# LukasHedegaard/continual-skeletons

Hardware: AMD Instinct MI355X
Metric: clips/sec (ST-GCN clip forward, NTU-60 shape; CoST-GCN online step reported under costgcn_online) (higher is better)
Workload: dtype f32

## Files before the change

### continual-skeletons_amd/csrc/tcn_wino.hip

```cpp
#include <type_traits>

#include "mfma_core.h"
#include "tcn_params.h"

namespace {

constexpr int WMT = 64;
constexpr int WNT = 128;
constexpr int WTAPS = 12;

template <int VT, int MW = 1>
constexpr int wino_ldb() { return ((2 * ((WNT / MW + VT - 2) / VT) + 10) * VT + 3) / 4 * 4; }

struct WStage12x64 {
    unsigned goff0, loff0, gstride;
    f32x4 v[6];
    __device__ __forceinline__ void setup(int Cpad, int Mpad, int tid) {
        goff0 = (unsigned)(((tid >> 7) * Cpad + ((tid >> 4) & 7)) * Mpad + (tid & 15) * 4);
        loff0 = (unsigned)(tid * 4);
        gstride = (unsigned)(2 * Cpad * Mpad);
    }
    __device__ __forceinline__ void issue_slot(int u, const float *__restrict__ chunk_base) {
        v[u] = *reinterpret_cast<const f32x4 *>(chunk_base + (size_t)u * gstride + goff0);
    }
    __device__ __forceinline__ void issue(const float *__restrict__ chunk_base) {
#pragma unroll
        for (int u = 0; u < 6; ++u) issue_slot(u, chunk_base);
    }
    template <int G>
    __device__ __forceinline__ void issue_part(const float *__restrict__ chunk_base) {
        issue_slot(2 * G, chunk_base);
        issue_slot(2 * G + 1, chunk_base);
    }
    __device__ __forceinline__ void commit(float *__restrict__ Wl) const {
#pragma unroll
        for (int u = 0; u < 6; ++u) *reinterpret_cast<f32x4 *>(Wl + u * (NTHREADS * 4) + loff0) = v[u];
    }
};

template <int NT>
struct WStageNx128 {
    unsigned goff0, loff0, gstride;
    f32x4 v[NT];
    __device__ __forceinline__ void setup(int Cpad, int Mpad, int tid) {
        goff0 = 4u * (unsigned)((tid >> 5) * Mpad + (tid & 31) * 4);
        loff0 = (unsigned)(tid * 4);
        gstride = (unsigned)(Cpad * Mpad);
    }
    __device__ __forceinline__ void issue_slot(int u, const float *__restrict__ chunk_base) {
        v[u] = *reinterpret_cast<const f32x4 *>(reinterpret_cast<const char *>(chunk_base + (size_t)u * gstride) + goff0);
    }
    __device__ __forceinline__ void issue(const float *__restrict__ chunk_base) {
#pragma unroll
        for (int u = 0; u < NT; ++u) issue_slot(u, chunk_base);
    }
    template <int G>
    __device__ __forceinline__ void issue_part(const float *__restrict__ chunk_base) {
        constexpr int lo = NT == 13 ? (G == 0 ? 0 : 3 * G + 1) : 4 * G, hi = NT == 13 ? 3 * G + 4 : 4 * G + 4;
#pragma unroll
        for (int u = lo; u < hi; ++u) issue_slot(u, chunk_base);
    }
    __device__ __forceinline__ void commit(float *__restrict__ Wl) const {
#pragma unroll
        for (int u = 0; u < NT; ++u) *reinterpret_cast<f32x4 *>(Wl + u * (KC * 128) + loff0) = v[u];
    }
};

struct WStageRes64 {
    unsigned goff0, loff0;
    f32x4 v;
    __device__ __forceinline__ void setup(int Mpad, int tid) {
        goff0 = (unsigned)(((tid >> 4) & 7) * Mpad + (tid & 15) * 4);
        loff0 = (unsigned)((tid & 127) * 4);
    }
    __device__ __forceinline__ void issue(const float *__restrict__ chunk_base) {
        v = *reinterpret_cast<const f32x4 *>(chunk_base + goff0);
    }
    __device__ __forceinline__ void commit(float *__restrict__ Wl) const { *reinterpret_cast<f32x4 *>(Wl + loff0) = v; }
};

struct WStageRes128 {
    unsigned goff0, loff0;
    f32x4 v;
    __device__ __forceinline__ void setup(int Mpad, int tid) {
        goff0 = (unsigned)((tid >> 5) * Mpad + (tid & 31) * 4);
        loff0 = (unsigned)(tid * 4);
    }
    __device__ __forceinline__ void issue(const float *__restrict__ chunk_base) {
        v = *reinterpret_cast<const f32x4 *>(chunk_base + goff0);
    }
    __device__ __forceinline__ void commit(float *__restrict__ Wl) const { *reinterpret_cast<f32x4 *>(Wl + loff0) = v; }
};

template <int VT, int G, int MW>
__device__ __forceinline__ void wino_group(const float *__restrict__ Wl, const float *__restrict__ Bl, int off, int l31, int kh,
                                           f32x16 (&acc)[4][2]) {
    constexpr int LDB = wino_ldb<VT, MW>(), MT = WMT * MW;
    const float *br = Bl + kh * LDB + off + 3 * G * VT;
    const float *wr = Wl + 4 * G * (KC * MT) + kh * MT + l31;
#pragma unroll
    for (int s = 0; s < KC / 2; ++s) {
        const float d0 = br[2 * s * LDB], d1 = br[2 * s * LDB + VT], d2 = br[2 * s * LDB + 2 * VT], d3 = br[2 * s * LDB + 3 * VT];
        const float b[4] = {d0 - d2, d1 + d2, d2 - d1, d1 - d3};
#pragma unroll
        for (int i = 0; i < 4; ++i) {
            const float a0 = wr[i * (KC * MT) + 2 * s * MT], a1 = wr[i * (KC * MT) + 2 * s * MT + 32];
            acc[i][0] = __builtin_amdgcn_mfma_f32_32x32x2f32(a0, b[i], acc[i][0], 0, 0, 0);
            acc[i][1] = __builtin_amdgcn_mfma_f32_32x32x2f32(a1, b[i], acc[i][1], 0, 0, 0);
        }
    }
}

template <int VT, int MW>
__device__ __forceinline__ void wino_valid_res_chunk(const float *__restrict__ Wl, const float *__restrict__ Bl, int off, int l31,
                                                     int kh, f32x16 (&acc)[4][2]) {
    constexpr int LDB = wino_ldb<VT, MW>(), MT = WMT * MW;
    const float *br = Bl + kh * LDB + off;
    const float *wr = Wl + kh * MT + l31;
#pragma unroll
    for (int s = 0; s < KC / 2; ++s) {
        const float d0 = br[2 * s * LDB], nd1 = -br[2 * s * LDB + VT];
        const float a0 = wr[2 * s * MT], a1 = wr[2 * s * MT + 32];
        acc[0][0] = __builtin_amdgcn_mfma_f32_32x32x2f32(a0, d0, acc[0][0], 0, 0, 0);
        acc[0][1] = __builtin_amdgcn_mfma_f32_32x32x2f32(a1, d0, acc[0][1], 0, 0, 0);
        acc[3][0] = __builtin_amdgcn_mfma_f32_32x32x2f32(a0, nd1, acc[3][0], 0, 0, 0);
        acc[3][1] = __builtin_amdgcn_mfma_f32_32x32x2f32(a1, nd1, acc[3][1], 0, 0, 0);
    }
}

template <int VT, bool RES, bool VALID = false>
__device__ __forceinline__ void wino_epilogue(const TcnParams &p, const f32x16 (&acc)[4][2], int m0, int q0, int qend, int seg,
                                              int wn, int l31, int kh, int jc, int vc) {
    const int T = p.Tout, TV = T * VT;
    const int TVR = VALID ? p.Tin * VT : TV;
    const bool qv = q0 + wn * 32 + l31 < qend;
    const bool odd_ok = 2 * jc + 1 < T;
    const unsigned p0 = (unsigned)(2 * jc * VT + vc);
    const unsigned b0 = 4u * (4u * (unsigned)kh * (unsigned)TV + p0);
    const unsigned b1 = odd_ok ? b0 + 4u * VT : b0;
    const unsigned kh16 = 16u * (unsigned)kh;
    const unsigned r0 = VALID ? 4u * (4u * (unsigned)kh * (unsigned)TVR + p0 + 4u * VT) : b0;
    const unsigned r1 = VALID ? (odd_ok ? r0 + 4u * VT : r0) : b1;
    const float *rseg = RES ? p.xres + (int64_t)seg * p.Cout * TVR : nullptr;
    float *oseg = p.out + (int64_t)seg * p.Cout * TV;
#pragma unroll
    for (int mi = 0; mi < 2; ++mi) {
        const int rb = m0 + mi * 32;
        float o0[16], o1[16];
#pragma unroll
        for (int g = 0; g < 16; ++g) {
            const int row = rb + (g & 3) + 8 * (g >> 2);
            const float bias = ld_lane(p.bias + row, kh16);
            const float m1 = acc[1][mi][g], m2 = acc[2][mi][g];
            float v0 = acc[0][mi][g] + m1 + m2 + bias;
            float v1 = m1 - m2 - acc[3][mi][g] + bias;
            if (RES) {
                const float *rrow = rseg + (int64_t)row * TVR;
                v0 += ld_lane(rrow, r0);
                v1 += ld_lane(rrow, r1);
            }
            if (p.relu) { v0 = relu_nan(v0); v1 = relu_nan(v1); }
            o0[g] = v0;
            o1[g] = v1;
        }
        if (qv) {
#pragma unroll
            for (int g = 0; g < 16; ++g) {
                float *orow = oseg + (int64_t)(rb + (g & 3) + 8 * (g >> 2)) * TV;
                st_lane(orow, b0, o0[g]);
                if (odd_ok) st_lane(orow, b1, o1[g]);
            }
        }
    }
}

}

template <int VT, bool RES = true, int MW = 1, bool VALID = false, bool RESCONV = false>
__global__ __launch_bounds__(NTHREADS, 2) void tcn_stage_wino_kernel(const TcnParams p) {
    static_assert(!RESCONV || (VALID && !RES), "the conv-residual phase is built for the valid form");
    constexpr int LDB = wino_ldb<VT, MW>(), MT = WMT * MW, NT = WNT / MW;
    constexpr int NJ = (LDB + 63) / 64;
    extern __shared__ __attribute__((aligned(16))) float smem[];
    float *Wl = smem;
    float *Bl = smem + WTAPS * KC * MT;

    const int tid = threadIdx.x, lane = tid & 63, wave = __builtin_amdgcn_readfirstlane(tid >> 6);
    const int l31 = lane & 31, kh = lane >> 5;
    const int wm = MW == 2 ? wave >> 1 : 0, wn = MW == 2 ? wave & 1 : wave;
    const unsigned wid = xcd_contiguous_id(blockIdx.x, gridDim.x);
    const int m0 = (int)(wid % p.mtiles) * MT, q0 = (int)((wid / p.mtiles) % p.qtiles) * NT;
    const int seg = (int)(wid / (p.mtiles * p.qtiles));
    const int T = VALID ? p.Tin : p.Tout, TV = T * VT, QP = p.nt;
    const int qend = min(q0 + NT, QP);
    const int ja = div_magic(q0, p.vmagic), jb = div_magic(qend - 1, p.vmagic);

    const int qc = min(q0 + wn * 32 + l31, qend - 1);
    const int jc = div_magic(qc, p.vmagic), vc = qc - jc * VT;
    const int off = 2 * (jc - ja) * VT + vc;

    f32x16 acc[4][2];
#pragma unroll
    for (int i = 0; i < 4; ++i)
#pragma unroll
        for (int mi = 0; mi < 2; ++mi)
#pragma unroll
            for (int g = 0; g < 16; ++g) acc[i][mi][g] = 0.f;

    {
        const int fa = VALID ? 2 * ja : 2 * ja - 4;
        const int span = (2 * (jb - ja) + 10) * VT;
        const int64_t cs = (int64_t)TV;
        const float *seg_base = p.y + (int64_t)seg * p.C * cs;
        const float *wbase = p.w + m0;
        const float *Ww = Wl + wm * WMT;
        std::conditional_t<MW == 2, WStageNx128<WTAPS>, WStage12x64> ws;
        ws.setup(p.Cpad, p.Mpad, tid);
        auto kloop = [&](auto &bx) {
            ws.issue(wbase);
            bx.issue(seg_base, p.C, cs, 0, wave);
            for (int c0 = 0; c0 + KC < p.Cpad; c0 += KC) {
                __syncthreads();
                ws.commit(Wl);
                bx.commit(Bl, LDB, wave);
                __syncthreads();
                const float *wnext = wbase + (size_t)(c0 + KC) * p.Mpad;
                const int cn = c0 + KC;
                ws.template issue_part<0>(wnext);
                bx.template issue_third<0>(seg_base, p.C, cs, cn, wave);
                __builtin_amdgcn_s_setprio(1);
                wino_group<VT, 0, MW>(Ww, Bl, off, l31, kh, acc);
                __builtin_amdgcn_s_setprio(0);
                ws.template issue_part<1>(wnext);
                bx.template issue_third<1>(seg_base, p.C, cs, cn, wave);
                __builtin_amdgcn_s_setprio(1);
                wino_group<VT, 1, MW>(Ww, Bl, off, l31, kh, acc);
                __builtin_amdgcn_s_setprio(0);
                ws.template issue_part<2>(wnext);
                bx.template issue_third<2>(seg_base, p.C, cs, cn, wave);
                __builtin_amdgcn_s_setprio(1);
                wino_group<VT, 2, MW>(Ww, Bl, off, l31, kh, acc);
                __builtin_amdgcn_s_setprio(0);
            }
            __syncthreads();
            ws.commit(Wl);
            bx.commit(Bl, LDB, wave);
            __syncthreads();
            wino_group<VT, 0, MW>(Ww, Bl, off, l31, kh, acc);
            wino_group<VT, 1, MW>(Ww, Bl, off, l31, kh, acc);
            wino_group<VT, 2, MW>(Ww, Bl, off, l31, kh, acc);
        };
        const bool interior = fa >= 0 && fa * VT + 4 * ((span + 3) / 4) <= TV;
        if (interior) {
            BStage4<(NJ + 3) / 4> b4;
            b4.setup(fa * VT, span, lane);
            kloop(b4);
        } else {
            BStage<NJ> bs;
            bs.setup(fa * VT, span, TV, lane);
            kloop(bs);
        }
    }

    if (RESCONV) {
        constexpr int NJ4R = (((2 * ((NT + VT - 2) / VT) + 2) * VT + 3) / 4 + 63) / 64;
        const int span = (2 * (jb - ja) + 2) * VT;
        const int64_t cs = (int64_t)p.Tres * VT;
        const float *seg_base = p.xres + (int64_t)seg * p.Cres * cs;
        const float *wbase = p.wres + m0;
        const float *Ww = Wl + wm * WMT;
        std::conditional_t<MW == 2, WStageRes128, WStageRes64> wr;
        wr.setup(p.Mpad, tid);
        BStage4<NJ4R> b4;
        b4.setup((2 * ja + 4) * VT, span, lane);
        wr.issue(wbase);
        b4.issue(seg_base, p.Cres, cs, 0, wave);
        for (int c0 = 0; c0 + KC < p.Cres; c0 += KC) {
            __syncthreads();
            wr.commit(Wl);
            b4.commit(Bl, LDB, wave);
            __syncthreads();
            wr.issue(wbase + (size_t)(c0 + KC) * p.Mpad);
            b4.issue(seg_base, p.Cres, cs, c0 + KC, wave);
            wino_valid_res_chunk<VT, MW>(Ww, Bl, off, l31, kh, acc);
        }
        __syncthreads();
        wr.commit(Wl);
        b4.commit(Bl, LDB, wave);
        __syncthreads();
        wino_valid_res_chunk<VT, MW>(Ww, Bl, off, l31, kh, acc);
    }

    wino_epilogue<VT, RES, VALID>(p, acc, m0 + wm * WMT, q0, qend, seg, wn, l31, kh, jc, vc);
}

namespace {

constexpr int W2TAPS = 13;

template <int VT, int MW = 1>
constexpr int wino2_ldb() { return ((4 * ((WNT / MW + VT - 2) / VT) + 11) * VT + 3) / 4 * 4; }

struct WStage13x64 {
    unsigned goff0, loff0, gstride, u6;
    f32x4 v[7];
    __device__ __forceinline__ void setup(int Cpad, int Mpad, int tid) {
        goff0 = (unsigned)(((tid >> 7) * Cpad + ((tid >> 4) & 7)) * Mpad + (tid & 15) * 4);
        loff0 = (unsigned)(tid * 4);
        gstride = (unsigned)(2 * Cpad * Mpad);
        u6 = tid >= 128 ? 5u : 6u;
    }
    __device__ __forceinline__ void issue_slot(int u, const float *__restrict__ chunk_base) {
        if (u < 6) v[u] = *reinterpret_cast<const f32x4 *>(chunk_base + (size_t)u * gstride + goff0);
        else v[6] = *reinterpret_cast<const f32x4 *>(chunk_base + (size_t)u6 * gstride + goff0);
    }
    __device__ __forceinline__ void issue(const float *__restrict__ chunk_base) {
#pragma unroll
        for (int u = 0; u < 7; ++u) issue_slot(u, chunk_base);
    }
    template <int G>
    __device__ __forceinline__ void issue_part(const float *__restrict__ chunk_base) {
        if (G < 3) {
            issue_slot(2 * G, chunk_base);
            issue_slot(2 * G + 1, chunk_base);
        } else {
            issue_slot(6, chunk_base);
        }
    }
    __device__ __forceinline__ void commit(float *__restrict__ Wl) const {
#pragma unroll
        for (int u = 0; u < 6; ++u) *reinterpret_cast<f32x4 *>(Wl + u * (NTHREADS * 4) + loff0) = v[u];
        *reinterpret_cast<f32x4 *>(Wl + u6 * (NTHREADS * 4) + loff0) = v[6];
    }
};

template <int LDB>
struct BStage4Tail {
    static constexpr int RPW = KC / (NTHREADS / 64);
    static constexpr int REST = LDB % 256;
    static constexpr int NV = LDB / 256 + (REST > 128 ? 1 : 0), NS = REST > 128 ? 0 : (REST + 63) / 64;
    static_assert(NV >= 1 && NV <= 2 && NS <= 2, "issue_third: 16-byte sweeps with thirds 0 and 1, 4-byte sweeps with third 2");
    unsigned off4[NV], off1[NS > 0 ? NS : 1];
    int pbase_;
    f32x4 v[RPW][NV];
    float t[RPW][NS > 0 ? NS : 1];
    __device__ __forceinline__ void setup(int pbase, int span, int lane) {
        const int nvec = (span + 3) / 4;
        pbase_ = pbase;
#pragma unroll
        for (int u = 0; u < NV; ++u) off4[u] = (unsigned)(4 * min(u * 64 + lane, nvec - 1));
#pragma unroll
        for (int u = 0; u < NS; ++u) off1[u] = (unsigned)min(NV * 256 + u * 64 + lane, span - 1);
    }
    __device__ __forceinline__ const float *row(const float *__restrict__ seg_base, int C, int64_t chan_stride, int c0, int wave,
                                                int rr) const {
        const int c = min(c0 + wave + rr * (NTHREADS / 64), C - 1);
        return seg_base + (int64_t)c * chan_stride + pbase_;
    }
    template <int G>
    __device__ __forceinline__ void issue_third(const float *__restrict__ seg_base, int C, int64_t chan_stride, int c0, int wave) {
#pragma unroll
        for (int rr = 0; rr < RPW; ++rr) {
            const float *src = row(seg_base, C, chan_stride, c0, wave, rr);
            if (G < NV) v[rr][G < NV ? G : 0] = *reinterpret_cast<const f32x4u *>(src + off4[G < NV ? G : 0]);
            if (G == 2) {
#pragma unroll
                for (int u = 0; u < NS; ++u) t[rr][u] = src[off1[u]];
            }
        }
    }
    __device__ __forceinline__ void issue(const float *__restrict__ seg_base, int C, int64_t chan_stride, int c0, int wave) {
        issue_third<0>(seg_base, C, chan_stride, c0, wave);
        issue_third<1>(seg_base, C, chan_stride, c0, wave);
        issue_third<2>(seg_base, C, chan_stride, c0, wave);
    }
    __device__ __forceinline__ void commit(float *__restrict__ Bl, int ldb, int wave) const {
#pragma unroll
        for (int rr = 0; rr < RPW; ++rr) {
            float *dst = Bl + (wave + rr * (NTHREADS / 64)) * ldb;
#pragma unroll
            for (int u = 0; u < NV; ++u) *reinterpret_cast<f32x4 *>(dst + off4[u]) = v[rr][u];
#pragma unroll
            for (int u = 0; u < NS; ++u) dst[off1[u]] = t[rr][u];
        }
    }
};

template <int VT, int ROW0, int F, int NP, int MW>
__device__ __forceinline__ void wino2_group(const float *__restrict__ Wl, const float *__restrict__ Bl, int off, int l31, int kh,
                                            f32x16 (&acc)[4][2]) {
    constexpr int LDB = wino2_ldb<VT, MW>(), MT = WMT * MW;
    const float *br = Bl + kh * LDB + off + F * VT;
    const float *wr = Wl + ROW0 * (KC * MT) + kh * MT + l31;
#pragma unroll
    for (int s = 0; s < KC / 2; ++s) {
        const float d0 = br[2 * s * LDB], d1 = br[2 * s * LDB + 2 * VT], d2 = br[2 * s * LDB + 4 * VT];
        const float d3 = NP == 4 ? br[2 * s * LDB + 6 * VT] : 0.f;
        const float b[4] = {d0 - d2, d1 + d2, d2 - d1, d1 - d3};
#pragma unroll
        for (int i = 0; i < NP; ++i) {
            const float a0 = wr[i * (KC * MT) + 2 * s * MT], a1 = wr[i * (KC * MT) + 2 * s * MT + 32];
            acc[i][0] = __builtin_amdgcn_mfma_f32_32x32x2f32(a0, b[i], acc[i][0], 0, 0, 0);
            acc[i][1] = __builtin_amdgcn_mfma_f32_32x32x2f32(a1, b[i], acc[i][1], 0, 0, 0);
        }
    }
}

template <int VT, int MW>
__device__ __forceinline__ void wino2_res_chunk(const float *__restrict__ Wl, const float *__restrict__ Bl, int off, int l31, int kh,
                                                f32x16 (&acc)[4][2]) {
    constexpr int LDB = wino2_ldb<VT, MW>(), MT = WMT * MW;
    const float *br = Bl + kh * LDB + off;
    const float *wr = Wl + kh * MT + l31;
#pragma unroll
    for (int s = 0; s < KC / 2; ++s) {
        const float d0 = br[2 * s * LDB], d1 = br[2 * s * LDB + 2 * VT];
        const float a0 = wr[2 * s * MT], a1 = wr[2 * s * MT + 32];
        const float b0 = d0 - d1;
        acc[0][0] = __builtin_amdgcn_mfma_f32_32x32x2f32(a0, b0, acc[0][0], 0, 0, 0);
        acc[0][1] = __builtin_amdgcn_mfma_f32_32x32x2f32(a1, b0, acc[0][1], 0, 0, 0);
        acc[1][0] = __builtin_amdgcn_mfma_f32_32x32x2f32(a0, d1, acc[1][0], 0, 0, 0);
        acc[1][1] = __builtin_amdgcn_mfma_f32_32x32x2f32(a1, d1, acc[1][1], 0, 0, 0);
    }
}

}

template <int VT, bool RESCONV, int MW = 1>
__global__ __launch_bounds__(NTHREADS, 2) void tcn_stage_wino_s2_kernel(const TcnParams p) {
    constexpr int LDB = wino2_ldb<VT, MW>(), MT = WMT * MW, NT = WNT / MW;
    constexpr int NJ = (LDB + 63) / 64;
    constexpr int NJR = ((4 * ((NT + VT - 2) / VT) + 3) * VT + 63) / 64;
    extern __shared__ __attribute__((aligned(16))) float smem[];
    float *Wl = smem;
    float *Bl = smem + W2TAPS * KC * MT;

    const int tid = threadIdx.x, lane = tid & 63, wave = __builtin_amdgcn_readfirstlane(tid >> 6);
    const int l31 = lane & 31, kh = lane >> 5;
    const int wm = MW == 2 ? wave >> 1 : 0, wn = MW == 2 ? wave & 1 : wave;
    const unsigned wid = xcd_contiguous_id(blockIdx.x, gridDim.x);
    const int m0 = (int)(wid % p.mtiles) * MT, q0 = (int)((wid / p.mtiles) % p.qtiles) * NT;
    const int seg = (int)(wid / (p.mtiles * p.qtiles));
    const int TVin = p.Tin * VT, QP = p.nt;
    const int qend = min(q0 + NT, QP);
    const int ja = div_magic(q0, p.vmagic), jb = div_magic(qend - 1, p.vmagic);
    const float *Ww = Wl + wm * WMT;

    const int qc = min(q0 + wn * 32 + l31, qend - 1);
    const int jc = div_magic(qc, p.vmagic), vc = qc - jc * VT;
    const int off = 4 * (jc - ja) * VT + vc;

    f32x16 acc[4][2];
#pragma unroll
    for (int i = 0; i < 4; ++i)
#pragma unroll
        for (int mi = 0; mi < 2; ++mi)
#pragma unroll
            for (int g = 0; g < 16; ++g) acc[i][mi][g] = 0.f;

    {
        const int fa = 4 * ja - 4;
        const int span = (4 * (jb - ja) + 11) * VT;
        const int64_t cs = (int64_t)TVin;
        const float *seg_base = p.y + (int64_t)seg * p.C * cs;
        const float *wbase = p.w + m0;
        std::conditional_t<MW == 2, WStageNx128<W2TAPS>, WStage13x64> ws;
        ws.setup(p.Cpad, p.Mpad, tid);
        auto kloop = [&](auto &bx) {
            ws.issue(wbase);
            bx.issue(seg_base, p.C, cs, 0, wave);
            for (int c0 = 0; c0 + KC < p.Cpad; c0 += KC) {
                __syncthreads();
                ws.commit(Wl);
                bx.commit(Bl, LDB, wave);
                __syncthreads();
                const float *wnext = wbase + (size_t)(c0 + KC) * p.Mpad;
                const int cn = c0 + KC;
                ws.template issue_part<0>(wnext);
                bx.template issue_third<0>(seg_base, p.C, cs, cn, wave);
                __builtin_amdgcn_s_setprio(1);
                wino2_group<VT, 0, 0, 4, MW>(Ww, Bl, off, l31, kh, acc);
                __builtin_amdgcn_s_setprio(0);
                ws.template issue_part<1>(wnext);
                bx.template issue_third<1>(seg_base, p.C, cs, cn, wave);
                __builtin_amdgcn_s_setprio(1);
                wino2_group<VT, 4, 6, 3, MW>(Ww, Bl, off, l31, kh, acc);
                __builtin_amdgcn_s_setprio(0);
                ws.template issue_part<2>(wnext);
                bx.template issue_third<2>(seg_base, p.C, cs, cn, wave);
                __builtin_amdgcn_s_setprio(1);
                wino2_group<VT, 7, 1, 3, MW>(Ww, Bl, off, l31, kh, acc);
                __builtin_amdgcn_s_setprio(0);
                ws.template issue_part<3>(wnext);
                __builtin_amdgcn_s_setprio(1);
                wino2_group<VT, 10, 5, 3, MW>(Ww, Bl, off, l31, kh, acc);
                __builtin_amdgcn_s_setprio(0);
            }
            __syncthreads();
            ws.commit(Wl);
            bx.commit(Bl, LDB, wave);
            __syncthreads();
            wino2_group<VT, 0, 0, 4, MW>(Ww, Bl, off, l31, kh, acc);
            wino2_group<VT, 4, 6, 3, MW>(Ww, Bl, off, l31, kh, acc);
            wino2_group<VT, 7, 1, 3, MW>(Ww, Bl, off, l31, kh, acc);
            wino2_group<VT, 10, 5, 3, MW>(Ww, Bl, off, l31, kh, acc);
        };
        const bool interior = fa >= 0 && fa * VT + 4 * ((span + 3) / 4) <= TVin;
        if (interior) {
            std::conditional_t<MW == 2, BStage4Tail<LDB>, BStage4<(NJ + 3) / 4>> b4;
            b4.setup(fa * VT, span, lane);
            kloop(b4);
        } else {
            BStage<NJ> bs;
            bs.setup(fa * VT, span, TVin, lane);
            kloop(bs);
        }
    }

    if (RESCONV) {
        const int span = (4 * (jb - ja) + 3) * VT;
        const int64_t cs = (int64_t)p.Tres * VT;
        const float *seg_base = p.xres + (int64_t)seg * p.Cres * cs;
        const float *wbase = p.wres + m0;
        const int cend = (p.Cres + KC - 1) / KC * KC;
        std::conditional_t<MW == 2, WStageRes128, WStageRes64> wr;
        wr.setup(p.Mpad, tid);
        BStage<NJR> bs;
        bs.setup(4 * ja * VT, span, p.Tres * VT, lane);
        wr.issue(wbase);
        bs.issue(seg_base, p.Cres, cs, 0, wave);
        for (int c0 = 0; c0 + KC < cend; c0 += KC) {
            __syncthreads();
            wr.commit(Wl);
            bs.commit(Bl, LDB, wave);
            __syncthreads();
            wr.issue(wbase + (size_t)(c0 + KC) * p.Mpad);
            bs.issue(seg_base, p.Cres, cs, c0 + KC, wave);
            wino2_res_chunk<VT, MW>(Ww, Bl, off, l31, kh, acc);
        }
        __syncthreads();
        wr.commit(Wl);
        bs.commit(Bl, LDB, wave);
        __syncthreads();
        wino2_res_chunk<VT, MW>(Ww, Bl, off, l31, kh, acc);
    }

    wino_epilogue<VT, false>(p, acc, m0 + wm * WMT, q0, qend, seg, wn, l31, kh, jc, vc);
}

static int wino_pick_mw(int qp, int c_out, int stride) {
    if (c_out % (2 * WMT) != 0) return 1;
    const int force = csk_diag_int("CSK_TCN_WINO");
    if (force == 2 || force == 3) return force - 1;
    if (stride == 2) return 2;
    const int64_t wide = round_up(qp, WNT), tall = round_up(qp, WNT / 2);
    return 16 * tall <= 15 * wide ? 2 : 1;
}

static int tcn_stage_wino_launch(const float *y, const float *w_wino, const float *x_res, const float *bias, float *out, int n_seg,
                                 int c, int c_out, int t_in, int V, int k, int stride, int pad, int res_mode, int c_res, int t_res,
                                 int res_off, int relu, void *stream, bool res_none = false) {
    if (!w_wino || !y || !bias || !out) return -2;
    if (k != 9 || stride != 1 || pad != 4) return -2;
    if (res_none ? res_mode != CSK_RES_NONE : (res_mode != CSK_RES_IDENTITY || res_off != 0 || !x_res || c_res != c_out || t_res != t_in))
        return -2;
    if ((V != 25 && V != 18) || c_out % WMT != 0 || c < 1 || n_seg < 1 || t_in < 1) return -2;
    if ((int64_t)t_in * V >= (1 << 26)) return -2;
    if (csk_diag_flag("CSK_TCN_WINO") && csk_diag_int("CSK_TCN_WINO") < 2) return -2;
    const int qp = (t_in + 1) / 2 * V;
    const int mw = wino_pick_mw(qp, c_out, stride);
    const int qtiles = (qp + WNT / mw - 1) / (WNT / mw), mtiles = c_out / (WMT * mw);
    if ((int64_t)qtiles * mtiles * n_seg >= (1ll << 31)) return -2;
    TcnParams p = {};
    p.y = y; p.w = w_wino; p.xres = res_none ? nullptr : x_res; p.wres = nullptr; p.bias = bias; p.out = out;
    p.C = c; p.Cpad = round_up(c, CSK_CPAD); p.Cout = c_out; p.Mpad = round_up(c_out, CSK_MT);
    p.Tin = t_in; p.Tout = t_in; p.V = V; p.K = k; p.stride = 1; p.pad = pad;
    p.res_mode = res_mode; p.Cres = res_none ? 0 : c_res; p.CresPad = round_up(p.Cres, CSK_CPAD); p.Tres = res_none ? 0 : t_res;
    p.res_off = 0; p.relu = relu;
    p.vmagic = vmagic_of(V); p.mtiles = (unsigned)mtiles; p.qtiles = (unsigned)qtiles; p.nt = qp;
    void (*kern)(TcnParams);
    int ldb;
    if (mw == 2) {
        kern = res_none ? (V == 25 ? tcn_stage_wino_kernel<25, false, 2> : tcn_stage_wino_kernel<18, false, 2>)
                        : (V == 25 ? tcn_stage_wino_kernel<25, true, 2> : tcn_stage_wino_kernel<18, true, 2>);
        ldb = V == 25 ? wino_ldb<25, 2>() : wino_ldb<18, 2>();
    } else {
        kern = res_none ? (V == 25 ? tcn_stage_wino_kernel<25, false> : tcn_stage_wino_kernel<18, false>)
                        : (V == 25 ? tcn_stage_wino_kernel<25> : tcn_stage_wino_kernel<18>);
        ldb = V == 25 ? wino_ldb<25>() : wino_ldb<18>();
    }
    p.ldb = ldb;
    const size_t lds = (size_t)(WTAPS * KC * WMT * mw + KC * ldb) * sizeof(float);
    if (const int e = csk_ensure_lds((const void *)kern, lds)) return e;
    hipLaunchKernelGGL(kern, dim3((unsigned)(qtiles * mtiles * n_seg)), dim3(NTHREADS), lds, (hipStream_t)stream, p);
    return (int)hipGetLastError();
}

static int tcn_stage_wino_valid_launch(const float *y, const float *w_wino, const float *x_res, const float *bias, float *out,
                                       int n_seg, int c, int c_out, int t_in, int V, int k, int stride, int pad, int res_mode,
                                       int c_res, int t_res, int res_off, int relu, void *stream, bool res_conv = false,
                                       const float *w_res = nullptr) {
    if (!w_wino || !y || !bias || !out) return -2;
    if (k != 9 || stride != 1 || pad != 0 || t_in < 9) return -2;
    const bool res = res_mode == CSK_RES_IDENTITY;
    if (res_conv ? res_mode != CSK_RES_CONV : (!res && res_mode != CSK_RES_NONE)) return -2;
    if (res && (res_off != 4 || !x_res || c_res != c_out || t_res != t_in)) return -2;
    if (res_conv && (res_off != 4 || !x_res || !w_res || c_res < CSK_CPAD || c_res % CSK_CPAD != 0 || t_res != t_in)) return -2;
    if ((V != 25 && V != 18) || c_out % WMT != 0 || c < 1 || n_seg < 1) return -2;
    if ((int64_t)t_in * V >= (1 << 26)) return -2;
    if (csk_diag_flag("CSK_TCN_WINO") && csk_diag_int("CSK_TCN_WINO") < 2) return -2;
    const int t_out = t_in - 8;
    const int qp = (t_out + 1) / 2 * V;
    const int mw = wino_pick_mw(qp, c_out, stride);
    const int qtiles = (qp + WNT / mw - 1) / (WNT / mw), mtiles = c_out / (WMT * mw);
    if ((int64_t)qtiles * mtiles * n_seg >= (1ll << 31)) return -2;
    const bool xr = res || res_conv;
    TcnParams p = {};
    p.y = y; p.w = w_wino; p.xres = xr ? x_res : nullptr; p.wres = res_conv ? w_res : nullptr; p.bias = bias; p.out = out;
    p.C = c; p.Cpad = round_up(c, CSK_CPAD); p.Cout = c_out; p.Mpad = round_up(c_out, CSK_MT);
    p.Tin = t_in; p.Tout = t_out; p.V = V; p.K = k; p.stride = 1; p.pad = 0;
    p.res_mode = res_mode; p.Cres = xr ? c_res : 0; p.CresPad = round_up(p.Cres, CSK_CPAD); p.Tres = xr ? t_res : 0;
    p.res_off = xr ? 4 : 0; p.relu = relu;
    p.vmagic = vmagic_of(V); p.mtiles = (unsigned)mtiles; p.qtiles = (unsigned)qtiles; p.nt = qp;
    void (*kern)(TcnParams);
    int ldb;
    if (mw == 2) {
        kern = res_conv ? (V == 25 ? tcn_stage_wino_kernel<25, false, 2, true, true> : tcn_stage_wino_kernel<18, false, 2, true, true>)
               : res    ? (V == 25 ? tcn_stage_wino_kernel<25, true, 2, true> : tcn_stage_wino_kernel<18, true, 2, true>)
                        : (V == 25 ? tcn_stage_wino_kernel<25, false, 2, true> : tcn_stage_wino_kernel<18, false, 2, true>);
        ldb = V == 25 ? wino_ldb<25, 2>() : wino_ldb<18, 2>();
    } else {
        kern = res_conv ? (V == 25 ? tcn_stage_wino_kernel<25, false, 1, true, true> : tcn_stage_wino_kernel<18, false, 1, true, true>)
               : res    ? (V == 25 ? tcn_stage_wino_kernel<25, true, 1, true> : tcn_stage_wino_kernel<18, true, 1, true>)
                        : (V == 25 ? tcn_stage_wino_kernel<25, false, 1, true> : tcn_stage_wino_kernel<18, false, 1, true>);
        ldb = V == 25 ? wino_ldb<25>() : wino_ldb<18>();
    }
    p.ldb = ldb;
    const size_t lds = (size_t)(WTAPS * KC * WMT * mw + KC * ldb) * sizeof(float);
    if (const int e = csk_ensure_lds((const void *)kern, lds)) return e;
    hipLaunchKernelGGL(kern, dim3((unsigned)(qtiles * mtiles * n_seg)), dim3(NTHREADS), lds, (hipStream_t)stream, p);
    return (int)hipGetLastError();
}

static int tcn_stage_wino_s2_launch(const float *y, const float *w_s2, const float *x_res, const float *w_res, const float *bias,
                                    float *out, int n_seg, int c, int c_out, int t_in, int V, int k, int stride, int pad,
                                    int res_mode, int c_res, int t_res, int res_off, int relu, void *stream) {
    if (!w_s2 || !y || !bias || !out) return -2;
    if (k != 9 || stride != 2 || pad != 4 || res_off != 0) return -2;
    const bool conv = res_mode == CSK_RES_CONV;
    if (!conv && res_mode != CSK_RES_NONE) return -2;
    if (conv && (!x_res || !w_res || c_res < 1 || t_res != t_in)) return -2;
    if ((V != 25 && V != 18) || c_out % WMT != 0 || c < 1 || n_seg < 1 || t_in < 1) return -2;
    if ((int64_t)t_in * V >= (1 << 26)) return -2;
    if (csk_diag_flag("CSK_TCN_WINO") && csk_diag_int("CSK_TCN_WINO") < 2) return -2;
    const int t_out = (t_in - 1) / 2 + 1;
    const int qp = (t_out + 1) / 2 * V;
    const int mw = wino_pick_mw(qp, c_out, stride);
    const int qtiles = (qp + WNT / mw - 1) / (WNT / mw), mtiles = c_out / (WMT * mw);
    if ((int64_t)qtiles * mtiles * n_seg >= (1ll << 31)) return -2;
    TcnParams p = {};
    p.y = y; p.w = w_s2; p.xres = conv ? x_res : nullptr; p.wres = conv ? w_res : nullptr; p.bias = bias; p.out = out;
    p.C = c; p.Cpad = round_up(c, CSK_CPAD); p.Cout = c_out; p.Mpad = round_up(c_out, CSK_MT);
    p.Tin = t_in; p.Tout = t_out; p.V = V; p.K = k; p.stride = 2; p.pad = pad;
    p.res_mode = res_mode; p.Cres = conv ? c_res : 0; p.CresPad = round_up(p.Cres, CSK_CPAD); p.Tres = conv ? t_res : 0;
    p.res_off = 0; p.relu = relu;
    p.vmagic = vmagic_of(V); p.mtiles = (unsigned)mtiles; p.qtiles = (unsigned)qtiles; p.nt = qp;
    void (*kern)(TcnParams);
    int ldb;
    if (mw == 2) {
        kern = conv ? (V == 25 ? tcn_stage_wino_s2_kernel<25, true, 2> : tcn_stage_wino_s2_kernel<18, true, 2>)
                    : (V == 25 ? tcn_stage_wino_s2_kernel<25, false, 2> : tcn_stage_wino_s2_kernel<18, false, 2>);
        ldb = V == 25 ? wino2_ldb<25, 2>() : wino2_ldb<18, 2>();
    } else {
        kern = conv ? (V == 25 ? tcn_stage_wino_s2_kernel<25, true> : tcn_stage_wino_s2_kernel<18, true>)
                    : (V == 25 ? tcn_stage_wino_s2_kernel<25, false> : tcn_stage_wino_s2_kernel<18, false>);
        ldb = V == 25 ? wino2_ldb<25>() : wino2_ldb<18>();
    }
    p.ldb = ldb;
    const size_t lds = (size_t)(W2TAPS * KC * WMT * mw + KC * ldb) * sizeof(float);
    if (const int e = csk_ensure_lds((const void *)kern, lds)) return e;
    hipLaunchKernelGGL(kern, dim3((unsigned)(qtiles * mtiles * n_seg)), dim3(NTHREADS), lds, (hipStream_t)stream, p);
    return (int)hipGetLastError();
}

extern "C" int csk_tcn_stage_wino_f32(const float *y, const float *w, const float *x_res, const float *w_res, const float *bias,
                                      float *out, int n_seg, int c, int c_out, int t_in, int V, int k, int stride, int pad,
                                      int res_mode, int c_res, int t_res, int res_off, int relu, const float *w_wino, void *stream) {
    const int rc = tcn_stage_wino_launch(y, w_wino, x_res, bias, out, n_seg, c, c_out, t_in, V, k, stride, pad, res_mode, c_res,
                                         t_res, res_off, relu, stream);
    if (rc != -2) return rc;
    return csk_tcn_stage_f32(y, w, x_res, w_res, bias, out, n_seg, c, c_out, t_in, V, k, stride, pad, res_mode, c_res, t_res,
                             res_off, relu, stream);
}

extern "C" int csk_tcn_stage_wino_ext_f32(const float *y, const float *w, const float *x_res, const float *w_res, const float *bias,
                                          float *out, int n_seg, int c, int c_out, int t_in, int V, int k, int stride, int pad,
                                          int res_mode, int c_res, int t_res, int res_off, int relu, const float *w_wino_ext,
                                          void *stream) {
    int rc = -2;
    if (stride == 1)
        rc = tcn_stage_wino_launch(y, w_wino_ext, nullptr, bias, out, n_seg, c, c_out, t_in, V, k, stride, pad, res_mode, c_res,
                                   t_res, res_off, relu, stream, true);
    else if (stride == 2)
        rc = tcn_stage_wino_s2_launch(y, w_wino_ext, x_res, w_res, bias, out, n_seg, c, c_out, t_in, V, k, stride, pad, res_mode,
                                      c_res, t_res, res_off, relu, stream);
    if (rc != -2) return rc;
    return csk_tcn_stage_f32(y, w, x_res, w_res, bias, out, n_seg, c, c_out, t_in, V, k, stride, pad, res_mode, c_res, t_res,
                             res_off, relu, stream);
}

extern "C" int csk_tcn_stage_wino_valid_f32(const float *y, const float *w, const float *x_res, const float *w_res, const float *bias,
                                            float *out, int n_seg, int c, int c_out, int t_in, int V, int k, int stride, int pad,
                                            int res_mode, int c_res, int t_res, int res_off, int relu, const float *w_wino,
                                            void *stream) {
    const int rc = tcn_stage_wino_valid_launch(y, w_wino, x_res, bias, out, n_seg, c, c_out, t_in, V, k, stride, pad, res_mode,
                                               c_res, t_res, res_off, relu, stream);
    if (rc != -2) return rc;
    return csk_tcn_stage_f32(y, w, x_res, w_res, bias, out, n_seg, c, c_out, t_in, V, k, stride, pad, res_mode, c_res, t_res,
                             res_off, relu, stream);
}

extern "C" int csk_tcn_stage_wino_valid_res_f32(const float *y, const float *x_res, const float *w_res, const float *bias, float *out,
                                                int n_seg, int c, int c_out, int t_in, int V, int k, int stride, int pad,
                                                int res_mode, int c_res, int t_res, int res_off, int relu, const float *w_wino,
                                                void *stream) {
    return tcn_stage_wino_valid_launch(y, w_wino, x_res, bias, out, n_seg, c, c_out, t_in, V, k, stride, pad, res_mode, c_res, t_res,
                                       res_off, relu, stream, true, w_res);
}
```

Measured before the change: 4346.

## Software-pipeline Winograd TCN inner loop with LDS prefetch, carried frames and sched barriers

Replaces the per-group Winograd MFMA loops in the stride-1 and stride-2 temporal conv kernels with one unified chunk routine. The routine prefetches weight fragments a fixed distance ahead of the MFMAs, carries an overlapping input frame between groups instead of re-reading it from LDS, and uses sched_group_barrier to interleave LDS reads with MFMAs. The residual chunk loops are likewise double-buffered. The aim is to hide LDS latency behind MFMA issue and cut redundant shared-memory reads, at the cost of more live registers, which could hurt occupancy or cause spills at launch_bounds 2.

```diff
diff --git a/continual-skeletons_amd/csrc/tcn_wino.hip b/continual-skeletons_amd/csrc/tcn_wino.hip
--- a/continual-skeletons_amd/csrc/tcn_wino.hip
+++ b/continual-skeletons_amd/csrc/tcn_wino.hip
@@ -92,40 +92,111 @@
     __device__ __forceinline__ void commit(float *__restrict__ Wl) const { *reinterpret_cast<f32x4 *>(Wl + loff0) = v; }
 };
 
-template <int VT, int G, int MW>
-__device__ __forceinline__ void wino_group(const float *__restrict__ Wl, const float *__restrict__ Bl, int off, int l31, int kh,
-                                           f32x16 (&acc)[4][2]) {
-    constexpr int LDB = wino_ldb<VT, MW>(), MT = WMT * MW;
-    const float *br = Bl + kh * LDB + off + 3 * G * VT;
-    const float *wr = Wl + 4 * G * (KC * MT) + kh * MT + l31;
-#pragma unroll
-    for (int s = 0; s < KC / 2; ++s) {
-        const float d0 = br[2 * s * LDB], d1 = br[2 * s * LDB + VT], d2 = br[2 * s * LDB + 2 * VT], d3 = br[2 * s * LDB + 3 * VT];
-        const float b[4] = {d0 - d2, d1 + d2, d2 - d1, d1 - d3};
+struct WinoGroupsS1 {
+    static constexpr int NG = 3, FS = 1;
+    static constexpr int row0(int g) { return 4 * g; }
+    static constexpr int frame0(int g) { return 3 * g; }
+    static constexpr int np(int) { return 4; }
+    static constexpr int carry(int g) { return g > 0 ? 3 : -1; }
+};
+struct WinoGroupsS2 {
+    static constexpr int NG = 4, FS = 2;
+    static constexpr int row0(int g) { return g == 0 ? 0 : 3 * g + 1; }
+    static constexpr int frame0(int g) { return g == 0 ? 0 : g == 1 ? 6 : g == 2 ? 1 : 5; }
+    static constexpr int np(int g) { return g == 0 ? 4 : 3; }
+    static constexpr int carry(int g) { return g == 1 ? 3 : g == 3 ? 2 : -1; }
+};
+
+template <int G>
+using group_c = std::integral_constant<int, G>;
+
+template <class GR, int VT, int LDB, int MT, int AD, bool CARRY, class Between>
+__device__ __forceinline__ void wino_chunk(const float *__restrict__ Wl, const float *__restrict__ Bl, int off, int l31, int kh,
+                                           f32x16 (&acc)[4][2], Between between) {
+    static_assert(AD >= 1 && AD <= 3, "a pair's fragment is read inside its own step or the one in front");
+    constexpr int NS = KC / 2, NSTEP = GR::NG * NS;
+    const float *br = Bl + kh * LDB + off;
+    const float *wr = Wl + kh * MT + l31;
+    float d[NSTEP][4], a[NSTEP][4][2], keep[NS];
+    auto read_d = [&](int t) {
+        const int g = t / NS, s = t % NS;
+        const float *p = br + 2 * s * LDB + GR::frame0(g) * VT;
+#pragma unroll
+        for (int f = 0; f < 4; ++f)
+            d[t][f] = CARRY && f == 0 && GR::carry(g) >= 0 ? keep[s] : f < GR::np(g) ? p[f * GR::FS * VT] : 0.f;
+        if (CARRY && g + 1 < GR::NG && GR::carry(g + 1) >= 0) keep[s] = d[t][GR::carry(g + 1)];
+    };
+    auto read_a = [&](int t, int j) {
+        const int n = GR::np(t / NS), tt = j < n ? t : t + 1, i = j < n ? j : j - n;
+        if (tt < NSTEP) {
+            const float *p = wr + (GR::row0(tt / NS) + i) * (KC * MT) + 2 * (tt % NS) * MT;
+            a[tt][i][0] = p[0];
+            a[tt][i][1] = p[32];
+        }
+    };
+    read_d(0);
+#pragma unroll
+    for (int j = 0; j < AD; ++j) read_a(0, j);
+#pragma unroll
+    for (int t = 0; t < NSTEP; ++t) {
+        const int g = t / NS;
+        if (t > 0) __builtin_amdgcn_sched_barrier(0);
+        const float b[4] = {d[t][0] - d[t][2], d[t][1] + d[t][2], d[t][2] - d[t][1], d[t][1] - d[t][3]};
 #pragma unroll
         for (int i = 0; i < 4; ++i) {
-            const float a0 = wr[i * (KC * MT) + 2 * s * MT], a1 = wr[i * (KC * MT) + 2 * s * MT + 32];
-            acc[i][0] = __builtin_amdgcn_mfma_f32_32x32x2f32(a0, b[i], acc[i][0], 0, 0, 0);
-            acc[i][1] = __builtin_amdgcn_mfma_f32_32x32x2f32(a1, b[i], acc[i][1], 0, 0, 0);
-        }
+            if (i < GR::np(g)) {
+                acc[i][0] = __builtin_amdgcn_mfma_f32_32x32x2f32(a[t][i][0], b[i], acc[i][0], 0, 0, 0);
+                acc[i][1] = __builtin_amdgcn_mfma_f32_32x32x2f32(a[t][i][1], b[i], acc[i][1], 0, 0, 0);
+                read_a(t, i + AD);
+                if (i == 1 && t + 1 < NSTEP) read_d(t + 1);
+            }
+        }
+        if (t == 0) __builtin_amdgcn_sched_group_barrier(0x100, AD + 2, 0);
+#pragma unroll
+        for (int i = 0; i < GR::np(g); ++i) {
+            __builtin_amdgcn_sched_group_barrier(0x008, 2, 0);
+            if (i == 1) __builtin_amdgcn_sched_group_barrier(0x100, 3, 0);
+            else __builtin_amdgcn_sched_group_barrier(0x100, 1, 0);
+        }
+        if (t + 1 < NSTEP && (t + 1) % NS == 0) {
+            if (g == 0) between(group_c<1>{});
+            else if (g == 1) between(group_c<2>{});
+            else if constexpr (GR::NG > 3) between(group_c<3>{});
+        }
+    }
+}
+
+template <int VT, int LDB, int MT, int FS, class Products>
+__device__ __forceinline__ void wino_res_steps(const float *__restrict__ Wl, const float *__restrict__ Bl, int off, int l31, int kh,
+                                               Products products) {
+    constexpr int NS = KC / 2;
+    const float *br = Bl + kh * LDB + off;
+    const float *wr = Wl + kh * MT + l31;
+    float d[2][2], a[2][2];
+    auto read = [&](int s, float (&dd)[2], float (&aa)[2]) {
+        dd[0] = br[2 * s * LDB];
+        dd[1] = br[2 * s * LDB + FS * VT];
+        aa[0] = wr[2 * s * MT];
+        aa[1] = wr[2 * s * MT + 32];
+    };
+    read(0, d[0], a[0]);
+#pragma unroll
+    for (int s = 0; s < NS; ++s) {
+        if (s + 1 < NS) read(s + 1, d[(s + 1) & 1], a[(s + 1) & 1]);
+        products(a[s & 1][0], a[s & 1][1], d[s & 1][0], d[s & 1][1]);
     }
 }
 
 template <int VT, int MW>
 __device__ __forceinline__ void wino_valid_res_chunk(const float *__restrict__ Wl, const float *__restrict__ Bl, int off, int l31,
                                                      int kh, f32x16 (&acc)[4][2]) {
-    constexpr int LDB = wino_ldb<VT, MW>(), MT = WMT * MW;
-    const float *br = Bl + kh * LDB + off;
-    const float *wr = Wl + kh * MT + l31;
-#pragma unroll
-    for (int s = 0; s < KC / 2; ++s) {
-        const float d0 = br[2 * s * LDB], nd1 = -br[2 * s * LDB + VT];
-        const float a0 = wr[2 * s * MT], a1 = wr[2 * s * MT + 32];
+    wino_res_steps<VT, wino_ldb<VT, MW>(), WMT * MW, 1>(Wl, Bl, off, l31, kh, [&](float a0, float a1, float d0, float d1) {
+        const float nd1 = -d1;
         acc[0][0] = __builtin_amdgcn_mfma_f32_32x32x2f32(a0, d0, acc[0][0], 0, 0, 0);
         acc[0][1] = __builtin_amdgcn_mfma_f32_32x32x2f32(a1, d0, acc[0][1], 0, 0, 0);
         acc[3][0] = __builtin_amdgcn_mfma_f32_32x32x2f32(a0, nd1, acc[3][0], 0, 0, 0);
         acc[3][1] = __builtin_amdgcn_mfma_f32_32x32x2f32(a1, nd1, acc[3][1], 0, 0, 0);
-    }
+    });
 }
 
 template <int VT, bool RES, bool VALID = false>
@@ -181,6 +252,8 @@
     static_assert(!RESCONV || (VALID && !RES), "the conv-residual phase is built for the valid form");
     constexpr int LDB = wino_ldb<VT, MW>(), MT = WMT * MW, NT = WNT / MW;
     constexpr int NJ = (LDB + 63) / 64;
+    constexpr int AD = 2;
+    constexpr bool CARRY = true;
     extern __shared__ __attribute__((aligned(16))) float smem[];
     float *Wl = smem;
     float *Bl = smem + WTAPS * KC * MT;
@@ -229,26 +302,19 @@
                 ws.template issue_part<0>(wnext);
                 bx.template issue_third<0>(seg_base, p.C, cs, cn, wave);
                 __builtin_amdgcn_s_setprio(1);
-                wino_group<VT, 0, MW>(Ww, Bl, off, l31, kh, acc);
-                __builtin_amdgcn_s_setprio(0);
-                ws.template issue_part<1>(wnext);
-                bx.template issue_third<1>(seg_base, p.C, cs, cn, wave);
-                __builtin_amdgcn_s_setprio(1);
-                wino_group<VT, 1, MW>(Ww, Bl, off, l31, kh, acc);
-                __builtin_amdgcn_s_setprio(0);
-                ws.template issue_part<2>(wnext);
-                bx.template issue_third<2>(seg_base, p.C, cs, cn, wave);
-                __builtin_amdgcn_s_setprio(1);
-                wino_group<VT, 2, MW>(Ww, Bl, off, l31, kh, acc);
+                wino_chunk<WinoGroupsS1, VT, LDB, MT, AD, CARRY>(Ww, Bl, off, l31, kh, acc, [&](auto g) {
+                    __builtin_amdgcn_s_setprio(0);
+                    ws.template issue_part<g()>(wnext);
+                    bx.template issue_third<g()>(seg_base, p.C, cs, cn, wave);
+                    __builtin_amdgcn_s_setprio(1);
+                });
                 __builtin_amdgcn_s_setprio(0);
             }
             __syncthreads();
             ws.commit(Wl);
             bx.commit(Bl, LDB, wave);
             __syncthreads();
-            wino_group<VT, 0, MW>(Ww, Bl, off, l31, kh, acc);
-            wino_group<VT, 1, MW>(Ww, Bl, off, l31, kh, acc);
-            wino_group<VT, 2, MW>(Ww, Bl, off, l31, kh, acc);
+            wino_chunk<WinoGroupsS1, VT, LDB, MT, AD, CARRY>(Ww, Bl, off, l31, kh, acc, [](auto) {});
         };
         const bool interior = fa >= 0 && fa * VT + 4 * ((span + 3) / 4) <= TV;
         if (interior) {
@@ -386,42 +452,16 @@
     }
 };
 
-template <int VT, int ROW0, int F, int NP, int MW>
-__device__ __forceinline__ void wino2_group(const float *__restrict__ Wl, const float *__restrict__ Bl, int off, int l31, int kh,
-                                            f32x16 (&acc)[4][2]) {
-    constexpr int LDB = wino2_ldb<VT, MW>(), MT = WMT * MW;
-    const float *br = Bl + kh * LDB + off + F * VT;
-    const float *wr = Wl + ROW0 * (KC * MT) + kh * MT + l31;
-#pragma unroll
-    for (int s = 0; s < KC / 2; ++s) {
-        const float d0 = br[2 * s * LDB], d1 = br[2 * s * LDB + 2 * VT], d2 = br[2 * s * LDB + 4 * VT];
-        const float d3 = NP == 4 ? br[2 * s * LDB + 6 * VT] : 0.f;
-        const float b[4] = {d0 - d2, d1 + d2, d2 - d1, d1 - d3};
-#pragma unroll
-        for (int i = 0; i < NP; ++i) {
-            const float a0 = wr[i * (KC * MT) + 2 * s * MT], a1 = wr[i * (KC * MT) + 2 * s * MT + 32];
-            acc[i][0] = __builtin_amdgcn_mfma_f32_32x32x2f32(a0, b[i], acc[i][0], 0, 0, 0);
-            acc[i][1] = __builtin_amdgcn_mfma_f32_32x32x2f32(a1, b[i], acc[i][1], 0, 0, 0);
-        }
-    }
-}
-
 template <int VT, int MW>
 __device__ __forceinline__ void wino2_res_chunk(const float *__restrict__ Wl, const float *__restrict__ Bl, int off, int l31, int kh,
                                                 f32x16 (&acc)[4][2]) {
-    constexpr int LDB = wino2_ldb<VT, MW>(), MT = WMT * MW;
-    const float *br = Bl + kh * LDB + off;
-    const float *wr = Wl + kh * MT + l31;
-#pragma unroll
-    for (int s = 0; s < KC / 2; ++s) {
-        const float d0 = br[2 * s * LDB], d1 = br[2 * s * LDB + 2 * VT];
-        const float a0 = wr[2 * s * MT], a1 = wr[2 * s * MT + 32];
+    wino_res_steps<VT, wino2_ldb<VT, MW>(), WMT * MW, 2>(Wl, Bl, off, l31, kh, [&](float a0, float a1, float d0, float d1) {
         const float b0 = d0 - d1;
         acc[0][0] = __builtin_amdgcn_mfma_f32_32x32x2f32(a0, b0, acc[0][0], 0, 0, 0);
         acc[0][1] = __builtin_amdgcn_mfma_f32_32x32x2f32(a1, b0, acc[0][1], 0, 0, 0);
         acc[1][0] = __builtin_amdgcn_mfma_f32_32x32x2f32(a0, d1, acc[1][0], 0, 0, 0);
         acc[1][1] = __builtin_amdgcn_mfma_f32_32x32x2f32(a1, d1, acc[1][1], 0, 0, 0);
-    }
+    });
 }
 
 }
@@ -430,6 +470,8 @@
 __global__ __launch_bounds__(NTHREADS, 2) void tcn_stage_wino_s2_kernel(const TcnParams p) {
     constexpr int LDB = wino2_ldb<VT, MW>(), MT = WMT * MW, NT = WNT / MW;
     constexpr int NJ = (LDB + 63) / 64;
+    constexpr int AD = 2;
+    constexpr bool CARRY = true;
     constexpr int NJR = ((4 * ((NT + VT - 2) / VT) + 3) * VT + 63) / 64;
     extern __shared__ __attribute__((aligned(16))) float smem[];
     float *Wl = smem;
@@ -479,31 +521,19 @@
                 ws.template issue_part<0>(wnext);
                 bx.template issue_third<0>(seg_base, p.C, cs, cn, wave);
                 __builtin_amdgcn_s_setprio(1);
-                wino2_group<VT, 0, 0, 4, MW>(Ww, Bl, off, l31, kh, acc);
-                __builtin_amdgcn_s_setprio(0);
-                ws.template issue_part<1>(wnext);
-                bx.template issue_third<1>(seg_base, p.C, cs, cn, wave);
-                __builtin_amdgcn_s_setprio(1);
-                wino2_group<VT, 4, 6, 3, MW>(Ww, Bl, off, l31, kh, acc);
-                __builtin_amdgcn_s_setprio(0);
-                ws.template issue_part<2>(wnext);
-                bx.template issue_third<2>(seg_base, p.C, cs, cn, wave);
-                __builtin_amdgcn_s_setprio(1);
-                wino2_group<VT, 7, 1, 3, MW>(Ww, Bl, off, l31, kh, acc);
-                __builtin_amdgcn_s_setprio(0);
-                ws.template issue_part<3>(wnext);
-                __builtin_amdgcn_s_setprio(1);
-                wino2_group<VT, 10, 5, 3, MW>(Ww, Bl, off, l31, kh, acc);
+                wino_chunk<WinoGroupsS2, VT, LDB, MT, AD, CARRY>(Ww, Bl, off, l31, kh, acc, [&](auto g) {
+                    __builtin_amdgcn_s_setprio(0);
+                    ws.template issue_part<g()>(wnext);
+                    if constexpr (g() < 3) bx.template issue_third<g()>(seg_base, p.C, cs, cn, wave);
+                    __builtin_amdgcn_s_setprio(1);
+                });
                 __builtin_amdgcn_s_setprio(0);
             }
             __syncthreads();
             ws.commit(Wl);
             bx.commit(Bl, LDB, wave);
             __syncthreads();
-            wino2_group<VT, 0, 0, 4, MW>(Ww, Bl, off, l31, kh, acc);
-            wino2_group<VT, 4, 6, 3, MW>(Ww, Bl, off, l31, kh, acc);
-            wino2_group<VT, 7, 1, 3, MW>(Ww, Bl, off, l31, kh, acc);
-            wino2_group<VT, 10, 5, 3, MW>(Ww, Bl, off, l31, kh, acc);
+            wino_chunk<WinoGroupsS2, VT, LDB, MT, AD, CARRY>(Ww, Bl, off, l31, kh, acc, [](auto) {});
         };
         const bool interior = fa >= 0 && fa * VT + 4 * ((span + 3) / 4) <= TVin;
         if (interior) {
```

Result: faster. 4398 (median of 6 runs) (+1.2%).
